# 1Jamie/HMSE

Hardware: AMD Instinct MI355X
Metric: ingest_GiB_per_s (higher is better)
Workload: dtype u8; 1 GPU; full ingest (FastCDC 2/8/32 KiB + SHA-256 dedupe + MinHash-128/LSH 4x32 + dictionary DEFLATE level-9 profile) over 10.00 GB wikipedia; total_bytes=9999220736, seg_size=4194304, collective=none

## Files before the change

hmse_amd/csrc/l1_deflate.hip:

```cpp
#include "common.h"
#include "blockops.h"
#include <stdio.h>
#include <stdlib.h>
#include <mutex>

namespace dfl {

constexpr int HB = 12;
constexpr int NBK = 1 << HB;
constexpr uint32_t MINM = 4, MAXM = 258, WMAX = 32768;

__device__ __forceinline__ uint32_t hash4(uint32_t x) { return (x * 0x9E3779B1u) >> (32 - HB); }

__device__ __forceinline__ uint32_t alignb(uint32_t hi, uint32_t lo, uint32_t sh) { return __builtin_amdgcn_alignbyte(hi, lo, sh); }
__device__ __forceinline__ uint32_t ld32a(const uint8_t* W, uint32_t off) {
  const uint32_t* w = (const uint32_t*)(W + (off & ~3u));
  return alignb(w[1], w[0], off);
}
__device__ __forceinline__ void ld64a(const uint8_t* W, uint32_t off, uint32_t& x0, uint32_t& x1) {
  const uint32_t* w = (const uint32_t*)(W + (off & ~3u));
  const uint32_t a = w[0], b = w[1], c = w[2];
  x0 = alignb(b, a, off); x1 = alignb(c, b, off);
}
__device__ __forceinline__ uint32_t sort_key(const uint8_t* W, uint32_t off) {
// ... 14 lines not shown
__device__ __forceinline__ uint32_t cur_get(const uint32_t* c, uint32_t h) { return (c[h >> 1] >> ((h & 1u) * 16u)) & 0xFFFFu; }
__device__ __forceinline__ uint32_t cur_inc(uint32_t* c, uint32_t h) {
  const uint32_t sh = (h & 1u) * 16u;
  return (atomicAdd(&c[h >> 1], 1u << sh) >> sh) & 0xFFFFu;
}

__device__ __forceinline__ void len_sym(uint32_t len, uint32_t& code, uint32_t& eb, uint32_t& ev) {
  if (len == 258) { code = 285; eb = 0; ev = 0; return; }
  const uint32_t l = len - 3;
  if (l < 8) { code = 257 + l; eb = 0; ev = 0; return; }
  const uint32_t e = (31 - __builtin_clz(l)) - 2;
  code = 257 + 4 * e + 4 + ((l >> e) & 3); eb = e; ev = l & ((1u << e) - 1);
}
__device__ __forceinline__ void dist_sym(uint32_t dist, uint32_t& code, uint32_t& eb, uint32_t& ev) {
  const uint32_t d = dist - 1;
  if (d < 4) { code = d; eb = 0; ev = 0; return; }
  const uint32_t hb = 31 - __builtin_clz(d), e = hb - 1;
  code = 2 * hb + ((d >> e) & 1); eb = e; ev = d & ((1u << e) - 1);
}
__device__ __forceinline__ uint32_t len_extra_bits(uint32_t code) {
  if (code < 265 || code == 285) return 0;
  return (code - 261) >> 2;
}
__device__ __forceinline__ uint32_t dist_extra_bits(uint32_t code) { return code < 4 ? 0 : (code >> 1) - 1; }
__device__ __forceinline__ uint32_t fixed_len(uint32_t s) { return s < 144 ? 8 : s < 256 ? 9 : s < 280 ? 7 : 8; }

__device__ __forceinline__ void wave_sync() {
  __builtin_amdgcn_fence(__ATOMIC_ACQ_REL, "wavefront");
  __builtin_amdgcn_wave_barrier();
}

template <int NT>
__device__ __forceinline__ uint32_t block_exclusive_scan_w(uint32_t v, uint32_t t, uint32_t* red, uint32_t* total) {
  const uint32_t lane = t & 63u, wave = uni32(t >> 6);
  const uint32_t inc = wave_incl_scan(v);
  if (lane == 63u) red[wave] = inc;
  __syncthreads();
  const uint32_t c = lane < (uint32_t)(NT / 64) ? red[lane] : 0u;
  const uint32_t ci = wave_incl_scan(c);
  __syncthreads();
  *total = (uint32_t)__builtin_amdgcn_readlane((int)ci, 63);
  return (uint32_t)__builtin_amdgcn_readlane((int)(ci - c), (int)wave) + inc - v;
}

template <int N>
struct HuffScratchT {
  uint32_t key[N];
  uint32_t sorted[N];
  uint32_t w[2 * N];
  uint16_t parent[2 * N];
  uint32_t cnt[32];
};
using HuffL = HuffScratchT<288>;
using HuffD = HuffScratchT<32>;

template <int NT, bool WQ>
struct Small {
  uint32_t lf[288], df[32];
  uint32_t red[NT / 64 + 1];
  uint32_t qhead;
  uint32_t ocnt[4];
  uint32_t otot[4];
  unsigned long long opk[1];
  struct { uint32_t ji, job, L, Dl; uint64_t c, cstart, rec_at, dstart; } nx;
  struct { uint64_t rec_at; } cur;
  uint32_t pexit[NT / 64], pexit2[NT / 64], pconv[NT / 64];
  uint8_t wtab[WQ ? NT : 64];
};

constexpr int align16(int v) { return (v + 15) & ~15; }

#ifndef HMSE_TCAP_S
#define HMSE_TCAP_S 10048
#define HMSE_TCAP_S2 13952
#define HMSE_TCAP_SG 17408
#define HMSE_TCAP_SG2 22976
#endif
constexpr int NT_S = 1024, TCAP_S = HMSE_TCAP_S, TCAP_S2 = HMSE_TCAP_S2, TCAP_SG = HMSE_TCAP_SG, TCAP_SG2 = HMSE_TCAP_SG2;
constexpr int NT_M = 1024, TCAP_SG3 = 32768;
#ifndef HMSE_NT_B
#define HMSE_NT_B 1024
#endif
constexpr int NT_B = HMSE_NT_B, TCAP_B = 65536, LCAP_B = 32768;

template <int NT, int TCAP, int LCAP_, bool LDSM, bool MDG = false, bool MLG = false, bool NOK = false>
struct Layout {
  static constexpr int LCAP = LCAP_;
  static constexpr int W_OFF = 0;
  static constexpr int W_SZ = align16(TCAP + 64);
  static constexpr int CUR_OFF = W_OFF + W_SZ;
  static constexpr int CUR_SZ = NBK * 2;
  static constexpr int MARK_OFF = CUR_OFF + CUR_SZ;
  static constexpr int MARK_SZ = align16(LCAP / 8 + 16);
  static constexpr int SMALL_OFF = MARK_OFF + MARK_SZ;
  static constexpr int SMALL_SZ = align16((int)sizeof(Small<NT, !LDSM>));
  static constexpr int A_OFF = SMALL_OFF + SMALL_SZ;
  static constexpr int A_SZ = LDSM ? align16(2 * TCAP + 80) : align16(LCAP + 80);
  static constexpr int MD_OFF = A_OFF + A_SZ;
  static constexpr int MD_SZ = (LDSM && !MDG) ? align16(2 * LCAP) : 0;
  static constexpr int ML_OFF = MD_OFF + MD_SZ;
  static constexpr int ML_SZ = (LDSM && !MLG) ? align16(LCAP) : 0;
  static constexpr int K_OFF = ML_OFF + ML_SZ;
  static constexpr int K_SZ = (LDSM && !NOK) ? align16(TCAP + 16) : 0;
  static constexpr int TOTAL = K_OFF + K_SZ;
  static_assert(TOTAL <= 160 * 1024, "one workgroup's LDS image must fit the CU's 160 KiB");
  static_assert(!(LDSM && TCAP <= TCAP_SG2) || TOTAL <= 80 * 1024, "classes S .. SG2 run two workgroups per CU");
  static_assert(sizeof(HuffL) + sizeof(HuffD) <= CUR_SZ, "Huffman scratch must fit the cursor table");
};

template <typename HS>
__device__ void huff_lengths_wave(const uint32_t* freq, uint32_t n, uint32_t limit, uint8_t* lens, HS* hs) {
  const uint32_t lane = lane_id();
  uint32_t used = 0;
  for (uint32_t b = 0; b < n; b += 64) {
    const uint32_t s = b + lane;
    used += (uint32_t)__builtin_popcountll(__ballot(s < n && freq[s] != 0));
  }
  uint32_t dummy0 = 0xFFFFFFFFu, dummy1 = 0xFFFFFFFFu;
  if (used == 0) { dummy0 = 0; dummy1 = 1; }
  else if (used == 1) dummy0 = freq[0] != 0 ? 1u : 0u;
  uint32_t m = 0;
  for (uint32_t b = 0; b < n; b += 64) {
    const uint32_t s = b + lane;
    uint32_t f = s < n ? freq[s] : 0u;
    if (s == dummy0 || s == dummy1) f = 1;
    if (s < n) lens[s] = 0;
    const bool u = f != 0;
    const uint64_t mask = __ballot(u);
    if (u) hs->key[m + (uint32_t)__builtin_popcountll(mask & lanemask_lt())] = (f << 9) | s;
    m += (uint32_t)__builtin_popcountll(mask);
  }
  wave_sync();
  for (uint32_t j = lane; j < m; j += 64) {
    const uint32_t kj = hs->key[j];
    uint32_t r = 0;
    for (uint32_t i = 0; i < m; i++) r += hs->key[i] < kj;
    hs->sorted[r] = kj;
    hs->w[r] = kj >> 9;
  }
  if (lane < 32) hs->cnt[lane] = 0;
  wave_sync();
  if (lane == 0) {
    constexpr uint32_t INF = 0xFFFFFFFFu;
    uint32_t li = 0, ii = m, ni = m;
    uint32_t wl = m ? hs->w[0] : INF, wi = INF;
    for (uint32_t step = 0; step + 1 < m; step++) {
      uint32_t pick0, pick1, v0, v1;
      {
        const bool tl = li < m && (ii >= ni || wl <= wi);
        if (tl) { pick0 = li++; v0 = wl; wl = li < m ? hs->w[li] : INF; }
        else { pick0 = ii++; v0 = wi; wi = ii < ni ? hs->w[ii] : INF; }
      }
      {
        const bool tl = li < m && (ii >= ni || wl <= wi);
        if (tl) { pick1 = li++; v1 = wl; wl = li < m ? hs->w[li] : INF; }
        else { pick1 = ii++; v1 = wi; wi = ii < ni ? hs->w[ii] : INF; }
      }
      hs->w[ni] = v0 + v1;
      hs->parent[pick0] = (uint16_t)ni; hs->parent[pick1] = (uint16_t)ni;
      if (ii == ni) wi = v0 + v1;
      ni++;
    }
  }
  wave_sync();
  const uint32_t root = 2 * m - 2;
  for (uint32_t j = lane; j < m; j += 64) {
// ... 34 lines not shown
#pragma unroll
  for (uint32_t b = 1; b <= 15; b++) { code = (code + (b > 1 ? uni32(cnt[b - 1]) : 0u)) << 1; run[b] = code; }
  for (uint32_t b0 = 0; b0 < n; b0 += 64) {
    const uint32_t s = b0 + lane;
    const uint32_t l = s < n ? lens[s] : 0u;
    uint32_t mycode = 0;
#pragma unroll
    for (uint32_t b = 1; b <= 15; b++) {
      const uint64_t mask = __ballot(l == b);
      if (l == b) mycode = run[b] + (uint32_t)__builtin_popcountll(mask & lanemask_lt());
      run[b] += (uint32_t)__builtin_popcountll(mask);
    }
    if (s < n) codes[s] = l ? (uint16_t)(__builtin_bitreverse32(mycode) >> (32 - l)) : (uint16_t)0;
  }
  wave_sync();
}

__device__ __forceinline__ void put_bits(uint32_t* out, uint32_t off, uint32_t v, uint32_t nb) {
  if (nb == 0) return;
  const uint32_t w = off >> 5, s = off & 31;
  atomicOr(&out[w], v << s);
  if (s + nb > 32) atomicOr(&out[w + 1], v >> (32 - s));
}

template <typename SM>
__device__ void rle_tree_wave(const uint8_t* l, uint32_t n, SM* sm, uint32_t tok_base, uint32_t* tok_end) {
  const uint32_t lane = lane_id();
  uint64_t starts[5];
  uint32_t val[5];
#pragma unroll
  for (int b = 0; b < 5; b++) {
    const uint32_t i = b * 64 + lane;
    const uint32_t v = i < n ? l[i] : 0xFFu;
    const uint32_t pv = (i > 0 && i < n) ? l[i - 1] : 0x1FFu;
    val[b] = v;
    starts[b] = __ballot(i < n && (i == 0 || v != pv));
  }
  uint32_t base = tok_base;
#pragma unroll
  for (int b = 0; b < 5; b++) {
    const uint32_t i = b * 64 + lane;
    const bool is_start = (starts[b] >> lane) & 1ull;
    uint32_t nxt = n;
    {
      bool found = false;
#pragma unroll
      for (int c = 0; c < 5; c++) {
        if (c < b) continue;
        uint64_t m = starts[c];
        if (c == b) m &= (lane == 63) ? 0ull : (~0ull << (lane + 1));
        if (!found && m) { nxt = c * 64 + (uint32_t)__builtin_ctzll(m); found = true; }
      }
    }
    const uint32_t v = val[b];
    uint32_t R = is_start ? nxt - i : 0u;
    uint32_t cnt = 0, full = 0, rem = 0;
    if (is_start) {
      if (v == 0) { full = R / 138; rem = R % 138; cnt = full + (rem >= 3 ? 1u : rem); }
      else { const uint32_t r1 = R - 1; full = r1 / 6; rem = r1 % 6; cnt = 1 + full + (rem >= 3 ? 1u : rem); }
    }
    const uint32_t inc = wave_incl_scan(cnt);
    const uint32_t tot = (uint32_t)__builtin_amdgcn_readlane((int)inc, 63);
    uint32_t at = base + inc - cnt;
    if (is_start) {
      if (v == 0) {
        for (uint32_t k = 0; k < full; k++) { sm->rle_sym[at] = 18; sm->rle_eb[at] = 7; sm->rle_ev[at] = 127; at++; }
        if (rem >= 11) { sm->rle_sym[at] = 18; sm->rle_eb[at] = 7; sm->rle_ev[at] = (uint8_t)(rem - 11); at++; }
        else if (rem >= 3) { sm->rle_sym[at] = 17; sm->rle_eb[at] = 3; sm->rle_ev[at] = (uint8_t)(rem - 3); at++; }
        else for (uint32_t k = 0; k < rem; k++) { sm->rle_sym[at] = 0; sm->rle_eb[at] = 0; sm->rle_ev[at] = 0; at++; }
      } else {
        sm->rle_sym[at] = (uint8_t)v; sm->rle_eb[at] = 0; sm->rle_ev[at] = 0; at++;
        for (uint32_t k = 0; k < full; k++) { sm->rle_sym[at] = 16; sm->rle_eb[at] = 2; sm->rle_ev[at] = 3; at++; }
        if (rem >= 3) { sm->rle_sym[at] = 16; sm->rle_eb[at] = 2; sm->rle_ev[at] = (uint8_t)(rem - 3); at++; }
        else for (uint32_t k = 0; k < rem; k++) { sm->rle_sym[at] = (uint8_t)v; sm->rle_eb[at] = 0; sm->rle_ev[at] = 0; at++; }
      }
    }
    base += tot;
  }
  *tok_end = base;
  wave_sync();
}

#ifdef HMSE_DFL_STAMPS
__device__ unsigned long long g_dfl_stamps[6][24];
__device__ unsigned long long g_enc_stamps[8];
#define STAMP(i) do { if (threadIdx.x == 0) { const unsigned long long now__ = clock64(); stamp_acc[i] += now__ - stamp_last; stamp_last = now__; } } while (0)
#else
#define STAMP(i) do { } while (0)
#endif

__host__ __device__ __forceinline__ uint32_t rec_ntok_off() { return 1280u; }
__host__ __device__ __forceinline__ uint32_t rec_tok_off() { return 1296u; }
__host__ __device__ __forceinline__ uint32_t rec_body(uint32_t L) { return 1296u + 4u * ((L + 3u) & ~3u); }
__host__ __device__ __forceinline__ uint32_t rec_slot_off(uint32_t L, uint32_t variant) { return variant ? rec_body(L) : rec_tok_off(); }
__host__ __device__ __forceinline__ uint32_t rec_size(uint32_t L, bool has_dict) { return (rec_body(L) + (has_dict ? L + 5u + 16u : 0u) + 255u) & ~255u; }

struct Args {
  const uint8_t* data; uint64_t n;
  const uint64_t* cuts; const uint64_t* chunk_ids; const int64_t* base; uint64_t n_sel;
  uint32_t depth;
  uint32_t base_is_chunk;
  const uint64_t* rec_off;
  uint8_t* recs;
  uint64_t rec_cap; uint32_t* status;
  uint32_t* len_full; uint32_t* len_delta;
  uint8_t* scratch; size_t scratch_stride;
  uint8_t* scratch2; size_t scratch2_stride;
  const uint32_t* jobs; const uint32_t* n_jobs; uint32_t* counter;
  unsigned long long* prof_ctr; uint32_t prof_slot;
};


typedef const __attribute__((address_space(4))) Args* KArgs;
__device__ __forceinline__ KArgs kargs() {
  KArgs p = (KArgs)__builtin_amdgcn_kernarg_segment_ptr();
  asm volatile("" : "+s"(p));
  return p;
}

struct Scratch {
  uint16_t S[65536]; uint8_t K[65536 + 16];
  uint16_t jumpA[32768 + 8];
};

template <int NT, int TCAP, int LCAP_, bool LDSM, bool MDG = false, bool MLG = false, bool NOK = false, bool DICT = false>
__global__ __launch_bounds__(NT, (LDSM ? (NT == 1024 && TCAP <= TCAP_SG2 ? 8 : 4) : 2)) void l1_deflate_kernel(Args) {
  using LY = Layout<NT, TCAP, LCAP_, LDSM, MDG, MLG, NOK>;
  constexpr int LCAP = LY::LCAP;
  extern __shared__ __attribute__((aligned(16))) uint8_t smem[];
  uint8_t* const W = smem + LY::W_OFF;
  uint32_t* const cur = (uint32_t*)(smem + LY::CUR_OFF);
  uint32_t* const mark = (uint32_t*)(smem + LY::MARK_OFF);
  Small<NT, !LDSM>& sm = *(Small<NT, !LDSM>*)(smem + LY::SMALL_OFF);
  auto scratch_wg = [&]() -> Scratch* { const KArgs a = kargs(); return (Scratch*)(a->scratch + (size_t)blockIdx.x * a->scratch_stride); };
  auto scratch2_wg = [&]() -> uint8_t* { const KArgs a = kargs(); return a->scratch2 + (size_t)blockIdx.x * a->scratch2_stride; };
  Scratch* const sc = LDSM ? nullptr : scratch_wg();
  uint16_t* const S = LDSM ? (uint16_t*)(smem + LY::A_OFF) : sc->S;
  uint16_t* const jump = LDSM ? (uint16_t*)(smem + LY::A_OFF) : sc->jumpA;
  uint8_t* const K = LDSM ? (uint8_t*)(smem + LY::K_OFF) : sc->K;
  auto n_jobs_now = [&]() -> uint32_t { return *kargs()->n_jobs; };
#if defined(HMSE_NO_ORD) || defined(HMSE_NO_SORT_ORD)
  constexpr bool SORT_ORD = false;
#else
  constexpr bool SORT_ORD = LDSM && !MLG && !DICT;
#endif
#if defined(HMSE_NO_ORD) || defined(HMSE_NO_DICT_ORD) || defined(HMSE_NO_DICT_POSLIST)
  constexpr bool POS_ORD = false;
#else
  constexpr bool POS_ORD = LDSM && DICT;
#endif
  static_assert(!POS_ORD || TCAP < 65536, "a rank waits in a match-distance slot");
  static_assert(!SORT_ORD || LY::ML_SZ >= NBK * 2, "the bucket starts wait in the match-length area during the sort");
  [[maybe_unused]] uint32_t* const starts = (uint32_t*)(smem + LY::ML_OFF);
#ifdef HMSE_DFL_STAMPS
  unsigned long long stamp_acc[24] = {0}, stamp_last = clock64();
#endif

  auto pf_fetch_sync = [&]() {
    const KArgs a = kargs();
    const uint32_t ji2 = atomicAdd(a->counter, 1u);
    sm.nx.ji = ji2;
    if (ji2 >= *a->n_jobs) return;
    const uint32_t job2 = a->jobs[ji2];
    const uint64_t k2 = job2 >> 1;
    const uint64_t c2 = a->chunk_ids ? a->chunk_ids[k2] : k2;
    const uint64_t cs = a->cuts[c2];
    sm.nx.job = job2; sm.nx.c = c2; sm.nx.cstart = cs; sm.nx.L = (uint32_t)(a->cuts[c2 + 1] - cs); sm.nx.rec_at = a->rec_off[k2];
    if constexpr (DICT) {
      const int64_t bsel = a->base[k2];
      const uint64_t bc = (a->chunk_ids && !a->base_is_chunk) ? a->chunk_ids[bsel] : (uint64_t)bsel;
      uint64_t ds = a->cuts[bc], dl = a->cuts[bc + 1] - ds;
      if (dl > WMAX) { ds += dl - WMAX; dl = WMAX; }
      sm.nx.dstart = ds; sm.nx.Dl = (uint32_t)dl;
    }
  };
  if (threadIdx.x == 0) pf_fetch_sync();
  for (;;) {
    uint32_t t = threadIdx.x;
    asm volatile("" : "+v"(t));
    const uint32_t lane = t & 63u, wave = t >> 6;
    __syncthreads();
    const uint32_t ji = uni32(sm.nx.ji);
    if (ji >= n_jobs_now()) break;
    STAMP(10);
    constexpr uint32_t variant = DICT ? 1u : 0u;
    const uint32_t L = uni32(sm.nx.L);
    const uint32_t Dl = variant ? uni32(sm.nx.Dl) : 0u;
    const uint32_t T = Dl + L;
    uint32_t pf_u = 0; uint64_t pf_a = 0, pf_b = 0, pf_c = 0;
    auto pf_stage = [&](int stg) {
      const KArgs a = kargs();
      const uint32_t n_jobs = *a->n_jobs;
      const bool valid = stg <= 1 || sm.nx.ji < n_jobs;
      switch (stg) {
        case 0: pf_u = atomicAdd(a->counter, 1u); break;
        case 1: sm.nx.ji = pf_u; pf_u = pf_u < n_jobs ? a->jobs[pf_u] : 0u; break;
        case 2: {
          sm.nx.job = pf_u;
          if (valid) { const uint64_t k2 = pf_u >> 1; pf_a = a->chunk_ids ? a->chunk_ids[k2] : k2; pf_b = a->rec_off[k2]; if (DICT) pf_c = (uint64_t)a->base[k2]; }
          break;
        }
        case 3: sm.nx.c = pf_a; sm.nx.rec_at = pf_b; if (DICT) sm.nx.dstart = pf_c; break;
        case 4:
          if (valid) {
            const uint64_t c2 = sm.nx.c;
            pf_a = a->cuts[c2]; pf_b = a->cuts[c2 + 1];
            if (DICT) { const uint64_t bsel = sm.nx.dstart; pf_c = (a->chunk_ids && !a->base_is_chunk) ? a->chunk_ids[bsel] : bsel; }
          }
          break;
        case 5:
          sm.nx.cstart = pf_a; sm.nx.L = (uint32_t)(pf_b - pf_a);
          if (DICT && valid) { const uint64_t bc = pf_c; pf_a = a->cuts[bc]; pf_b = a->cuts[bc + 1]; }
          break;
        default:
          if (DICT && valid) { uint64_t ds = pf_a, dl = pf_b - pf_a; if (dl > WMAX) { ds += dl - WMAX; dl = WMAX; } sm.nx.dstart = ds; sm.nx.Dl = (uint32_t)dl; }
          break;
      }
    };
#define PF_STAGE(n) do { if (t == 0) pf_stage(n); } while (0)
    auto mdist_of = [&]() -> uint16_t* { if constexpr (LDSM && !MDG) return (uint16_t*)(smem + LY::MD_OFF); else return (uint16_t*)scratch2_wg(); };
    auto mlen_of = [&]() -> uint8_t* { if constexpr (LDSM && !MLG) return (uint8_t*)(smem + LY::ML_OFF); else return scratch2_wg() + 2u * (uint32_t)LCAP; };
    {
      const KArgs a = kargs();
      const uint64_t rec_at = uni64(sm.nx.rec_at);
      if (L > (uint32_t)LCAP || T > (uint32_t)TCAP || rec_at + (uint64_t)rec_size(L, variant != 0) > a->rec_cap) {
        if (t == 0) {
          const uint64_t k = sm.nx.job >> 1;
          (variant ? a->len_delta : a->len_full)[k] = 0xFFFFFFFFu;
          if (L <= 32768u) atomicOr(a->status, 2u);
        }
        __syncthreads();
        if (t == 0) pf_fetch_sync();
        continue;
      }
      if (t == 0) sm.cur.rec_at = rec_at;
    }
    const uint8_t* const csrc = kargs()->data + uni64(sm.nx.cstart);
    const uint8_t* const dsrc = kargs()->data + (variant ? uni64(sm.nx.dstart) : 0ull);
// ... 73 lines not shown
    STAMP(1);
    PF_STAGE(1);
    {
      static_assert(!SORT_ORD || TCAP < 65536, "16-bit list cursors");
      [[maybe_unused]] const uint16_t* const start_of = (const uint16_t*)starts;
      uint32_t q = t, h = 0, before = 0, hx = 0;
      [[maybe_unused]] uint32_t bidx = 0;
      bool act = q < nh;
      if (act) {
        hx = sort_key(W, q); h = hx >> (32 - HB); before = cur_get(cur, h);
        if constexpr (SORT_ORD) bidx = before - start_of[h];
      }
      [[maybe_unused]] uint32_t* ord = nullptr;
      [[maybe_unused]] uint32_t dcap = 0, ob1 = 0, ob2 = 0, ob3 = 0;
      if constexpr (SORT_ORD) {
        ord = (uint32_t*)(scratch2_wg() + 98304u);
        dcap = __builtin_elementwise_min(kargs()->depth, 63u);
        ob1 = uni32(sm.otot[0]); ob2 = ob1 + uni32(sm.otot[1]); ob3 = ob2 + uni32(sm.otot[2]);
      }
      [[maybe_unused]] uint16_t* rank_at = nullptr;
      if constexpr (POS_ORD) rank_at = mdist_of();
      __syncthreads();
      for (uint32_t q0 = 0; q0 < nh; q0 += NT) {
        if (act) S[cur_inc(cur, h)] = (uint16_t)q;
        __syncthreads();
        uint32_t r = 0;
        if (act) {
          const uint32_t after = cur_get(cur, h);
          for (uint32_t jj = before; jj < after; jj++) r += S[jj] < q;
        }
        [[maybe_unused]] uint32_t km = 0, obl = 0, obh = 0;
        [[maybe_unused]] uint64_t oc0 = 0, oc1 = 0, oc2 = 0, oc3 = 0;
        if constexpr (SORT_ORD) {
          km = bidx + r;
          km = km < dcap ? km : dcap;
          oc0 = __ballot(km >= 24u); oc1 = __ballot(km >= 12u); oc2 = __ballot(km >= 4u); oc3 = __ballot(km >= 1u);
          if (oc3 != 0 && lane == 0u) {
            uint32_t z = 0;
            asm volatile("" : "+v"(z));
            const unsigned long long got = atomicAdd(&sm.opk[z], (unsigned long long)__builtin_popcountll(oc0) | ((unsigned long long)__builtin_popcountll(oc1 & ~oc0) << 16) |
                                                                     ((unsigned long long)__builtin_popcountll(oc2 & ~oc1) << 32) | ((unsigned long long)__builtin_popcountll(oc3 & ~oc2) << 48));
            obl = (uint32_t)got; obh = (uint32_t)(got >> 32);
          }
        }
        const uint32_t qn = q0 + NT + t;
        const bool actn = qn < nh;
        uint32_t hn = 0, beforen = 0, hxn = 0;
        [[maybe_unused]] uint32_t bidxn = 0;
        if (actn) {
          hxn = sort_key(W, qn); hn = hxn >> (32 - HB); beforen = cur_get(cur, hn);
          if constexpr (SORT_ORD) bidxn = beforen - start_of[hn];
        }
        __syncthreads();
        if (act) { S[before + r] = (uint16_t)q; if constexpr (!NOK) K[before + r] = (uint8_t)((hx & 0x0Fu) | ((hx >> 12) & 0xF0u)); }
        if constexpr (POS_ORD) if (act && q >= Dl) *(uint16_t*)((uint8_t*)rank_at + ((q - Dl) << 1)) = (uint16_t)(before + r);
        if constexpr (SORT_ORD) {
          if (oc3 != 0) {
            const uint32_t gl = (uint32_t)__builtin_amdgcn_readlane((int)obl, 0), gh = (uint32_t)__builtin_amdgcn_readlane((int)obh, 0);
            uint32_t pos = 0;
            if (km >= 1u) { pos = ob3 + (gh >> 16) + mbcnt64(oc3 & ~oc2); asm volatile("" : "+v"(pos)); }
            if (km >= 4u) { pos = ob2 + (gh & 0xFFFFu) + mbcnt64(oc2 & ~oc1); asm volatile("" : "+v"(pos)); }
            if (km >= 12u) { pos = ob1 + (gl >> 16) + mbcnt64(oc1 & ~oc0); asm volatile("" : "+v"(pos)); }
            if (km >= 24u) { pos = (gl & 0xFFFFu) + mbcnt64(oc0); asm volatile("" : "+v"(pos)); }
            if (km != 0u) *(uint32_t*)((uint8_t*)ord + (pos << 2)) = (before + r) | (km << 15) | ((hx << 5) & 0x01E00000u);
          }
          bidx = bidxn;
        }
        q = qn; act = actn; h = hn; before = beforen; hx = hxn;
      }
      if constexpr (SORT_ORD) for (uint32_t i = t * 16; i < L; i += NT * 16) *(uint4*)(mlen0 + i) = make_uint4(0, 0, 0, 0);
      __syncthreads();
#ifdef HMSE_DIAG
      if constexpr (SORT_ORD) if (t < 4u && (uint32_t)((sm.opk[0] >> (16u * t)) & 0xFFFFull) != sm.otot[t]) atomicOr(kargs()->status, 32u);
#endif
    }
    STAMP(2);
    PF_STAGE(2);
    uint32_t* const anch = mark;
    uint8_t* const anchb = (uint8_t*)(mark + (LCAP / 64 + 2));
    static_assert(LCAP % 64 == 0 && (LCAP / 64 + 2) * 4 + LCAP / 64 + 2 <= LY::MARK_SZ, "anchors and their backward extents share the mark area");
    if constexpr (DICT) {
      const uint32_t n_anch = (L + 63u) >> 6;
      if (t < 2u) { anch[n_anch + t] = 0; anchb[n_anch + t] = 0; }
      for (uint32_t a0 = wave; a0 < n_anch; a0 += NT / 64) {
        const uint32_t pa = Dl + (a0 << 6);
        uint32_t word = 0, back = 0;
        if (pa + 4 <= T) {
          const uint32_t h = hash4(ld32a(W, pa));
          const uint32_t lo = h ? cur_get(cur, h - 1) : 0u, hi = cur_get(cur, h);
          uint32_t l = lo, r = hi;
          while (l < r) { const uint32_t m = (l + r) >> 1; if ((uint32_t)S[m] < Dl) l = m + 1; else r = m; }
          const uint32_t first = l > lo + 64u ? l - 64u : lo;
          const uint32_t idx = first + lane;
          uint32_t ml = 0, q = 0;
          if (idx < l) {
            q = S[idx];
            if (TCAP <= (int)WMAX || pa - q <= WMAX) {
              uint64_t qa[4], pb[4];
              ldNa<4>(W, q, qa); ldNa<4>(W, pa, pb);
              ml = 32;
#pragma unroll
              for (int u = 3; u >= 0; u--) { const uint64_t x = qa[u] ^ pb[u]; if (x) ml = 8u * u + ((uint32_t)__builtin_ctzll(x) >> 3); }
            }
          }
          uint32_t key = (ml << 8) | lane;
          key = wave_max(key);
          if ((key >> 8) >= 32u) {
            const uint32_t d = pa - (uint32_t)__builtin_amdgcn_readlane((int)q, (int)(key & 63u));
            const uint32_t off = 8u * lane;
            uint32_t n = 8;
            if (pa + off < T) {
              uint64_t xa[1], xb[1];
              ldNa<1>(W, pa + off - d, xa); ldNa<1>(W, pa + off, xb);
              const uint64_t x = xa[0] ^ xb[0];
              if (x) n = (uint32_t)__builtin_ctzll(x) >> 3;
            } else n = 0;
            const uint64_t mm = __ballot(n < 8u);
            uint32_t run = 512;
            if (mm) { const uint32_t fl = (uint32_t)__builtin_ctzll(mm); run = 8u * fl + (uint32_t)__builtin_amdgcn_readlane((int)n, (int)fl); }
            if (run > T - pa) run = T - pa;
            word = d | (run << 16);
            const uint32_t qa0 = pa - d;
            uint32_t nb = 8;
            if (lane < 16u) {
              nb = 0;
              if (qa0 >= off + 8u) {
                uint64_t ya[1], yb[1];
                ldNa<1>(W, qa0 - off - 8u, ya); ldNa<1>(W, pa - off - 8u, yb);
                const uint64_t y = ya[0] ^ yb[0];
                nb = y ? (uint32_t)__builtin_clzll(y) >> 3 : 8u;
              }
            }
            const uint64_t mb = __ballot(nb < 8u);
            back = 128;
            if (mb) {
              const uint32_t fl = (uint32_t)__builtin_ctzll(mb);
              const uint64_t n0 = __ballot((nb & 1u) != 0), n1 = __ballot((nb & 2u) != 0), n2 = __ballot((nb & 4u) != 0);
              back = 8u * fl + (uint32_t)((n0 >> fl) & 1ull) + 2u * (uint32_t)((n1 >> fl) & 1ull) + 4u * (uint32_t)((n2 >> fl) & 1ull);
            }
            if (back > (a0 << 6)) back = a0 << 6;
          }
        }
        anch[a0] = word; anchb[a0] = (uint8_t)back;
      }
      __syncthreads();
      STAMP(22);
    }
    auto hint_of = [&](uint32_t p, uint32_t maxlen, uint32_t& bq) -> uint32_t {
      const uint32_t a0 = (p - Dl) >> 6;
      uint32_t bm = 0; bq = 0;
#pragma unroll
      for (uint32_t back = 0; back < 2; back++) {
        if (a0 < back) continue;
        const uint32_t w = anch[a0 - back];
        const uint32_t d = w & 0xFFFFu, run = w >> 16, pa = Dl + ((a0 - back) << 6);
        if (w == 0 || p < pa || d > p || p - d >= Dl) continue;
        uint32_t m = 0;
        if (run >= 512u) m = maxlen;
        else if (pa + run > p) m = (pa + run - p) < maxlen ? (pa + run - p) : maxlen;
        if (m > bm) { bm = m; bq = p - d; }
      }
      return bm;
    };
    [[maybe_unused]] auto hint_word = [&](uint32_t p, uint32_t maxlen, uint32_t w, uint32_t pa, uint32_t& bm, uint32_t& bq) {
      const uint32_t d = w & 0xFFFFu, run = w >> 16;
      if (w == 0 || p < pa || d > p || p - d >= Dl) return;
      uint32_t m = 0;
      if (run >= 512u) m = maxlen;
      else if (pa + run > p) m = (pa + run - p) < maxlen ? (pa + run - p) : maxlen;
      if (m > bm) { bm = m; bq = p - d; }
    };
    [[maybe_unused]] auto known_of = [&](uint32_t p, uint32_t maxlen) -> uint32_t {
      const uint32_t a1 = ((p - Dl) >> 6) + 1u;
      uint32_t kf = 0;
#pragma unroll
      for (uint32_t f = 0; f < 2; f++) {
        const uint32_t w = anch[a1 + f], bk = anchb[a1 + f], pa = Dl + ((a1 + f) << 6);
        if (pa - p <= bk) {
          const uint32_t d = w & 0xFFFFu, run = w >> 16;
          uint32_t m = pa + run - p;
          if (run >= 512u || m > maxlen) m = maxlen;
          const uint32_t v = (p - d) | (m << 16);
          if (v > kf) kf = v;
        }
      }
      return kf;
    };
    if constexpr (DICT && !POS_ORD) {
      uint8_t* const mlen = mlen_of(); uint16_t* const mdist = mdist_of();
      for (uint32_t x = t; x < L; x += NT) {
        const uint32_t p = Dl + x;
        if (p + 4 > T) continue;
        const uint32_t maxlen = (T - p) < MAXM ? (T - p) : MAXM;
        uint32_t bq;
        const uint32_t bm = hint_of(p, maxlen, bq);
        if (bm >= 16u) { mlen[x] = (uint8_t)(bm - 3); mdist[x] = (uint16_t)(p - bq); }
      }
      if constexpr (!MLG && LDSM) __syncthreads();
      STAMP(23);
    }
#if defined(HMSE_NO_ORD)
    constexpr bool ORD = false;
#elif defined(HMSE_NO_DICT_ORD)
    constexpr bool ORD = !DICT && LDSM;
#else
    constexpr bool ORD = LDSM;
#endif
    auto ord_of = [&]() -> uint32_t* { return (uint32_t*)(scratch2_wg() + 98304u); };
    if constexpr (ORD && !SORT_ORD) {
      const uint32_t depth = kargs()->depth;
      uint32_t* const ord = ord_of();
      constexpr int ITER = (TCAP + NT - 1) / NT;
      const uint32_t wv = uni32(wave);
      constexpr int NPK = (ITER + 2) / 3;
      uint32_t pk[NPK];
#pragma unroll
      for (int w = 0; w < NPK; w++) pk[w] = 0;
      uint32_t n0 = 0, n1 = 0, n2 = 0, n3 = 0;
      if constexpr (!POS_ORD) {
        const uint32_t last = nh ? nh - 1u : 0u;
        constexpr int G = DICT ? 2 : ITER > 12 ? 4 : 8;
        [[maybe_unused]] const uint8_t* const mlen_h = mlen_of();
#pragma unroll
        for (int g = 0; g < ITER; g += G) if ((uint32_t)g * NT < nh) {
          uint32_t pv[G], hv[G], lv[G];
#pragma unroll
          for (int u = 0; u < G; u++) if (g + u < ITER) { const uint32_t r = (wv << 6) + (uint32_t)(g + u) * NT + lane; pv[u] = S[r < last ? r : last]; }
#pragma unroll
          for (int u = 0; u < G; u++) if (g + u < ITER) hv[u] = ld32a(W, pv[u]) * 0x9E3779B1u;
// ... 499 lines not shown
          mark[wb >> 5] = (uint32_t)m; mark[(wb >> 5) + 1] = (uint32_t)(m >> 32);
        }
        conv_out = conv;
        return conv ? chain_exit : curp;
      };
      {
        const uint32_t sw = wave * SEG;
        bool conv = true;
        uint32_t ex = sm.pexit[wave];
        if (wave > 0 && sw < L) ex = stitch(wave, sm.pexit[wave - 1], sm.pexit[wave], true, conv);
        wave_sync();
        sm.pexit2[wave] = ex; sm.pconv[wave] = (wave == 0 || sw >= L || conv) ? 1u : 0u;
      }
      __syncthreads();
      if (wave == 0) {
        uint32_t first_bad = NW;
        for (uint32_t w = 0; w < NW; w++) if (sm.pconv[w] == 0u) { first_bad = w; break; }
        if (first_bad < NW) {
          uint32_t tru = sm.pexit2[first_bad];
          for (uint32_t w = first_bad + 1; w < NW; w++) {
            if (w * SEG >= L) break;
            bool cv;
            tru = stitch(w, tru, sm.pexit2[w], false, cv);
          }
        }
      }
    }
    __syncthreads();
    STAMP(4);
    PF_STAGE(6);
    {
      const KArgs a = kargs();
      uint8_t* const rec_c = a->recs + uni64(sm.cur.rec_at);
      const uint16_t* const mdist_c = mdist_of();
      uint32_t* const tok = (uint32_t*)(rec_c + rec_tok_off());
      const uint32_t ppt = (L + NT - 1) / NT;
      const uint32_t p0 = t * ppt < L ? t * ppt : L, p1 = (p0 + ppt) < L ? (p0 + ppt) : L;
      auto bits_at = [&](uint32_t pos, uint32_t nb) -> uint32_t {
        const uint32_t w = pos >> 5;
        const uint64_t v = (uint64_t)mark[w] | ((uint64_t)mark[w + 1] << 32);
        return (uint32_t)(v >> (pos & 31u)) & (nb >= 32u ? 0xFFFFFFFFu : ((1u << nb) - 1u));
      };
      uint32_t cntm = 0;
      for (uint32_t pos = p0; pos < p1; pos += 32) cntm += (uint32_t)__builtin_popcount(bits_at(pos, p1 - pos));
      uint32_t ntok;
      uint32_t idx = block_exclusive_scan_w<NT>(cntm, t, sm.red, &ntok);
      for (uint32_t pos = p0; pos < p1; pos += 32) {
        uint32_t m = bits_at(pos, p1 - pos);
        while (m) {
          const uint32_t x = pos + (uint32_t)__builtin_ctz(m);
          m &= m - 1;
          uint32_t l3 = 0;
          bool tk;
          if constexpr (LDSM) { const uint32_t nxj = jump[x]; tk = nxj > x + 1u; l3 = nxj - x - 3u; }
          else { tk = take(x); if (tk) l3 = mlen_c[x]; }
          if (tk) {
            const uint32_t dd = mdist_c[x];
            uint32_t code, eb, ev;
            len_sym(l3 + 3u, code, eb, ev); atomicAdd(&sm.lf[code], 1u);
            dist_sym(dd, code, eb, ev); atomicAdd(&sm.df[code], 1u);
            tok[idx] = (256u + l3) | (dd << 16);
          } else {
            const uint32_t b = W[Dl + x];
            atomicAdd(&sm.lf[b], 1u);
            tok[idx] = b;
          }
          idx++;
        }
      }
      if (t == 0) { atomicAdd(&sm.lf[256], 1u); *(uint32_t*)(rec_c + rec_ntok_off()) = ntok; if (a->prof_ctr) atomicAdd(&a->prof_ctr[a->prof_slot], (unsigned long long)ntok); }
      __syncthreads();
      STAMP(5);
      uint32_t* const r_hist = (uint32_t*)rec_c;
      for (uint32_t i = t; i < 288; i += NT) r_hist[i] = sm.lf[i];
      if (t < 32) r_hist[288 + t] = sm.df[t];
    }
    STAMP(9);
#ifdef HMSE_DFL_STAMPS
    if (t == 0) { stamp_acc[14] += L; stamp_acc[15]++; }
#endif
  }
#undef PF_STAGE
#ifdef HMSE_DFL_STAMPS
  if (threadIdx.x == 0) for (int i = 0; i < 24; i++) atomicAdd(&g_dfl_stamps[(TCAP <= TCAP_S ? 0 : TCAP <= TCAP_SG ? 1 : 2) + (DICT ? 3 : 0)][i], stamp_acc[i]);
#endif
}


struct EncSmall {
  uint32_t lf[288], df[32], cf[20];
  uint8_t ll[288], dl[32], cl[20];
  uint16_t lc[288], dc[32], cc[20];
  uint8_t rle_sym[352], rle_eb[352], rle_ev[352];
  uint32_t nr, nlit, ndist, ncl, mode, hdr_bits, fixed_bits, extra_bits, data_bits, cl_bits;
  uint32_t job, spill;
};
template <int LMIN_, int LCAP_>
struct EncLayout {
  static constexpr int NT = 128, LMIN = LMIN_, LCAP = LCAP_;
  static constexpr int NB_MAX = (LCAP + 63) / 64;
  static constexpr int NBLK = (NB_MAX + 1 + 63) / 64;
  static constexpr int SMALL_OFF = 0;
  static constexpr int SMALL_SZ = align16((int)sizeof(EncSmall));
  static constexpr int HS_OFF = SMALL_OFF + SMALL_SZ;
  static constexpr int HS_SZ = align16((int)(sizeof(HuffL) + sizeof(HuffD)));
  static constexpr int TT_OFF = HS_OFF;
  static constexpr int OUT_OFF = TT_OFF + 2048;
  static constexpr int WIN_BYTES = 4096;
  static constexpr int OUT_SZ = HS_SZ - 2048;
  static constexpr bool BOFF_IN_LF = NB_MAX + 1 <= 288;
  static constexpr int BOFF_OFF = HS_OFF + HS_SZ;
  static constexpr int BOFF_SZ = BOFF_IN_LF ? 0 : align16(4 * (NB_MAX + 1));
  static constexpr int TOTAL = BOFF_OFF + BOFF_SZ;
  static_assert(OUT_SZ >= WIN_BYTES + 64, "window + overhang");
  static_assert(LCAP > 12288 || TOTAL <= 10240, "sixteen workgroups per CU for the records of chunks <= 12 KiB");
};

template <int LMIN, int LCAP>
__global__ __launch_bounds__(128, 8) void l1_encode_kernel(Args a, const bool force_spill) {
  using EL = EncLayout<LMIN, LCAP>;
  constexpr uint32_t NT = EL::NT;
  constexpr uint32_t WIN_BITS = EL::WIN_BYTES * 8;
  extern __shared__ __attribute__((aligned(16))) uint8_t smem[];
  EncSmall& sm = *(EncSmall*)(smem + EL::SMALL_OFF);
  HuffL* const hsL = (HuffL*)(smem + EL::HS_OFF);
  HuffD* const hsD = (HuffD*)(smem + EL::HS_OFF + sizeof(HuffL));
  uint32_t* const TT = (uint32_t*)(smem + EL::TT_OFF);
  uint32_t* const out = (uint32_t*)(smem + EL::OUT_OFF);
  uint32_t* const boff = EL::BOFF_IN_LF ? sm.lf : (uint32_t*)(smem + EL::BOFF_OFF);
  const uint32_t n_jobs = *a.n_jobs;
#ifdef HMSE_DFL_STAMPS
  unsigned long long e_acc0 = 0, e_acc1 = 0, e_acc2 = 0, e_acc3 = 0, e_acc4 = 0, e_acc5 = 0, e_n = 0, e_last = clock64();
#define ESTAMP(v) do { if (threadIdx.x == 0) { const unsigned long long now__ = clock64(); v += now__ - e_last; e_last = now__; } } while (0)
#else
#define ESTAMP(v) do { } while (0)
#endif
  for (;;) {
  uint32_t t = threadIdx.x;
  asm volatile("" : "+v"(t));
  const uint32_t lane = t & 63u, wave = uni32(t >> 6);
  __syncthreads();
  if (t == 0) sm.job = atomicAdd(a.counter, 1u);
  __syncthreads();
  const uint32_t ji = uni32(sm.job);
  if (ji >= n_jobs) break;
  const uint32_t job = uni32(a.jobs[ji]);
  const uint64_t k = job >> 1;
  const uint32_t variant = job & 1u;
  const uint64_t c = a.chunk_ids ? uni64(a.chunk_ids[k]) : k;
  const uint64_t cstart = uni64(a.cuts[c]);
  const uint32_t L = uni32((uint32_t)(a.cuts[c + 1] - cstart));
  if (L <= (uint32_t)LMIN || L > (uint32_t)LCAP) continue;
  uint32_t* len_out = variant ? a.len_delta : a.len_full;
  if (uni32(len_out[k]) == 0xFFFFFFFFu) continue;
  uint8_t* const rec = a.recs + uni64(a.rec_off[k]);
  const uint32_t* const r_hist = (const uint32_t*)rec;
  const uint32_t ntok = uni32(*(const uint32_t*)(rec + rec_ntok_off()));
  const uint32_t* const tok = (const uint32_t*)(rec + rec_tok_off());
  if (a.prof_ctr && t == 0) atomicAdd(&a.prof_ctr[a.prof_slot], (unsigned long long)ntok);
  uint8_t* const slot = rec + rec_slot_off(L, variant);
  const uint8_t* const lit = a.data + cstart;
  for (uint32_t i = t; i < 288; i += NT) sm.lf[i] = r_hist[i];
  if (t < 32) sm.df[t] = r_hist[288 + t];
  if (t < 20) sm.cf[t] = 0;
  __syncthreads();
  ESTAMP(e_acc0);
  if (wave == 0) huff_lengths_wave(sm.lf, 286, 15, sm.ll, hsL);
// ... 372 lines not shown
  if (n_dev) n = *n_dev;
  __shared__ unsigned long long s[SC_NT / 64];
  const uint64_t i = (uint64_t)blockIdx.x * SC_NT + threadIdx.x;
  unsigned long long v = i < n ? in[i] : 0ull;
  for (int d = 32; d > 0; d >>= 1) v += __shfl_down(v, d, 64);
  if (lane_id() == 0) s[threadIdx.x >> 6] = v;
  __syncthreads();
  if (threadIdx.x == 0) { unsigned long long tt = 0; for (int w = 0; w < SC_NT / 64; w++) tt += s[w]; bsum[blockIdx.x] = tt; }
}
__global__ __launch_bounds__(SC_NT) void scan_apply_kernel(const uint64_t* __restrict__ in, uint64_t n, const uint64_t* __restrict__ bsum,
                                                            uint64_t* __restrict__ out, const uint64_t* __restrict__ n_dev) {
  if (n_dev) n = *n_dev;
  __shared__ unsigned long long s[SC_NT / 64];
  const uint64_t i = (uint64_t)blockIdx.x * SC_NT + threadIdx.x;
  const unsigned long long v = i < n ? in[i] : 0ull;
  const unsigned long long inc = wave_incl_scan((uint64_t)v);
  if (lane_id() == 63) s[threadIdx.x >> 6] = inc;
  __syncthreads();
  unsigned long long wb = 0;
  for (uint32_t w = 0; w < (threadIdx.x >> 6); w++) wb += s[w];
  if (i < n) out[i] = bsum[blockIdx.x] + wb + inc - v;
  if (i + 1 == n) out[n] = bsum[blockIdx.x] + wb + inc;
}

static int exclusive_scan_u64(const uint64_t* in, uint64_t n, uint64_t* out, uint64_t* bsum, uint64_t* total, hipStream_t stream,
                              const uint64_t* n_dev = nullptr) {
  const uint64_t nb = (n + SC_NT - 1) / SC_NT;
  scan_reduce_kernel<<<dim3((uint32_t)nb), dim3(SC_NT), 0, stream>>>(in, n, bsum, n_dev);
  block_sums_scan_kernel<SC_NT, 0, uint64_t, SC_NT><<<dim3(1), dim3(SC_NT), 0, stream>>>(bsum, nb, total, n_dev);
  scan_apply_kernel<<<dim3((uint32_t)nb), dim3(SC_NT), 0, stream>>>(in, n, bsum, out, n_dev);
  return hipGetLastError() == hipSuccess ? HMSE_OK : HMSE_EHIP;
}

constexpr int N_WG_B = 256;

struct Ws {
  uint32_t* counters;
  uint64_t* rec_off; uint64_t* final_len; uint64_t* bsum; uint64_t* rec_total;
  uint32_t* len_full; uint32_t* len_delta; uint32_t* lists; uint64_t list_stride;
  uint8_t* scratch; uint8_t* scratch2; uint8_t* recs; size_t fixed_bytes;
};
static Ws carve(void* ws, uint64_t n_sel) {
  WsCarver w(ws, ~(size_t)0);
  Ws r;
  r.counters = w.take<uint32_t>(N_CTR);
  r.rec_total = w.take<uint64_t>(1);
  r.rec_off = w.take<uint64_t>(n_sel + 1);
  r.final_len = w.take<uint64_t>(n_sel + 1);
  r.bsum = w.take<uint64_t>((n_sel + SC_NT - 1) / SC_NT + 1);
  r.len_full = w.take<uint32_t>(n_sel);
  r.len_delta = w.take<uint32_t>(n_sel);
  r.list_stride = 2 * n_sel;
  r.lists = w.take<uint32_t>(N_LIST * r.list_stride);
  r.scratch = w.take<uint8_t>((size_t)N_WG_B * hmse_align_up(sizeof(Scratch), 256));
  r.scratch2 = w.take<uint8_t>((size_t)512 * hmse_align_up(8 * 32768, 256));
  r.fixed_bytes = w.off;
  r.recs = r.scratch ? (uint8_t*)ws + w.off : nullptr;
  return r;
}

template <bool DICT, int NT, int TCAP, int LCAP, bool LDSM, bool MDG = false, bool MLG = false, bool NOK = false>
static int launch_class(Args a, uint32_t grid, hipStream_t stream) {
  using LY = Layout<NT, TCAP, LCAP, LDSM, MDG, MLG, NOK>;
  static std::once_flag attr_once;
  static hipError_t attr_rc = hipSuccess;
  std::call_once(attr_once, [] {
    attr_rc = hipFuncSetAttribute((const void*)l1_deflate_kernel<NT, TCAP, LCAP, LDSM, MDG, MLG, NOK, DICT>, hipFuncAttributeMaxDynamicSharedMemorySize, LY::TOTAL);
  });
  if (attr_rc != hipSuccess) return HMSE_EHIP;
  l1_deflate_kernel<NT, TCAP, LCAP, LDSM, MDG, MLG, NOK, DICT><<<dim3(grid), dim3(NT), LY::TOTAL, stream>>>(a);
  return hipGetLastError() == hipSuccess ? HMSE_OK : HMSE_EHIP;
}

}

#ifdef HMSE_DFL_STAMPS
extern "C" int hmse_debug_encode_stamps(unsigned long long* out8, int reset) {
  if (hipMemcpyFromSymbol(out8, HIP_SYMBOL(dfl::g_enc_stamps), sizeof(dfl::g_enc_stamps)) != hipSuccess) return HMSE_EHIP;
  if (reset) { unsigned long long z[8] = {0}; if (hipMemcpyToSymbol(HIP_SYMBOL(dfl::g_enc_stamps), z, sizeof z) != hipSuccess) return HMSE_EHIP; }
  return HMSE_OK;
}
extern "C" int hmse_debug_deflate_stamps(unsigned long long* out96, int reset) {
  if (hipMemcpyFromSymbol(out96, HIP_SYMBOL(dfl::g_dfl_stamps), sizeof(dfl::g_dfl_stamps)) != hipSuccess) return HMSE_EHIP;
  if (reset) { unsigned long long z[144] = {0}; if (hipMemcpyToSymbol(HIP_SYMBOL(dfl::g_dfl_stamps), z, sizeof z) != hipSuccess) return HMSE_EHIP; }
  return HMSE_OK;
}
#endif

extern "C" uint64_t hmse_l1_deflate_record_bytes(uint32_t chunk_len) { return chunk_len <= 32768u ? dfl::rec_size(chunk_len, false) : 0u; }
extern "C" uint64_t hmse_l1_deflate_record_bytes_dict(uint32_t chunk_len) { return chunk_len <= 32768u ? dfl::rec_size(chunk_len, true) : 0u; }

size_t hmse_l1_deflate_workspace_bytes_impl(uint64_t n_sel, const hmse_cfg*) { return dfl::carve(nullptr, n_sel).fixed_bytes; }

static int deflate_impl(const uint8_t* data, uint64_t n, const uint64_t* cuts, const uint64_t* chunk_ids,
                        const int64_t* base, uint64_t n_sel, const uint64_t* n_dev, const uint64_t* out_base_dev, const hmse_cfg* cfg, uint32_t flags,
                        uint8_t* out, uint64_t out_cap, uint64_t* out_off, uint8_t* kind, uint32_t* status, void* ws, size_t ws_bytes,
                        void* stream_);

extern "C" int hmse_l1_deflate_ex(const uint8_t* data, uint64_t n, const uint64_t* cuts, const uint64_t* chunk_ids,
                                  const int64_t* base, uint64_t n_sel, const hmse_cfg* cfg, uint32_t flags, uint8_t* out,
                                  uint64_t out_cap, uint64_t* out_off, uint8_t* kind, uint32_t* status, void* ws, size_t ws_bytes,
                                  void* stream_) {
  return deflate_impl(data, n, cuts, chunk_ids, base, n_sel, nullptr, nullptr, cfg, flags, out, out_cap, out_off, kind, status, ws, ws_bytes, stream_);
}

int hmse_l1_deflate_dyn(const uint8_t* data, uint64_t n_cap, const uint64_t* cuts_all, const uint64_t* sel_ids, const int64_t* sel_base,
                        const uint64_t* n_sel_dev, uint64_t cap_sel, const uint64_t* out_base_dev, const hmse_cfg* cfg, uint8_t* out, uint64_t out_cap,
                        uint64_t* out_off, uint8_t* kind, uint32_t* status, void* ws, size_t ws_bytes, hipStream_t stream) {
  if (!n_sel_dev || cap_sel == 0) return HMSE_EINVAL;
  return deflate_impl(data, n_cap, cuts_all, sel_ids, sel_base, cap_sel, n_sel_dev, out_base_dev, cfg, HMSE_DEFLATE_BASE_IS_CHUNK_ID, out, out_cap, out_off,
                      kind, status, ws, ws_bytes, (void*)stream);
}

static int deflate_impl(const uint8_t* data, uint64_t n, const uint64_t* cuts, const uint64_t* chunk_ids,
                        const int64_t* base, uint64_t n_sel, const uint64_t* n_dev, const uint64_t* out_base_dev, const hmse_cfg* cfg, uint32_t flags,
                        uint8_t* out, uint64_t out_cap, uint64_t* out_off, uint8_t* kind, uint32_t* status, void* ws, size_t ws_bytes,
                        void* stream_) {
  HMSE_WS_ALIGNED(ws);
  using namespace dfl;
  if (hmse_cfg_validate_impl(cfg) != 0) return HMSE_EINVAL;
  if (flags & ~(uint32_t)HMSE_DEFLATE_BASE_IS_CHUNK_ID) return HMSE_EINVAL;
  const uint32_t a_base_is_chunk = (flags & HMSE_DEFLATE_BASE_IS_CHUNK_ID) ? 1u : 0u;
  if (!out_off || !status) return HMSE_EINVAL;
  hipStream_t stream = (hipStream_t)stream_;
  (void)hipGetLastError();
  HMSE_FILL(status, 0, sizeof(uint32_t), stream);
  if (n_sel == 0) { HMSE_FILL(out_off, 0, sizeof(uint64_t), stream); return HMSE_OK; }
  if (!data || !cuts || !out || !kind) return HMSE_EINVAL;
  if (n_sel > 0x3FFFFFFFull) return HMSE_EINVAL;
  Ws w = carve(ws, n_sel);
  if (!ws || ws_bytes < w.fixed_bytes) return HMSE_ENOSPC;
  const uint64_t avail = ws_bytes - w.fixed_bytes;
  HMSE_FILL(w.counters, 0, N_CTR * sizeof(uint32_t), stream);
  HMSE_FILL(w.len_full, 0, n_sel * sizeof(uint32_t), stream);
  HMSE_FILL(w.len_delta, 0, n_sel * sizeof(uint32_t), stream);
  const uint32_t blocks = (uint32_t)((n_sel + 255) / 256);
  rec_size_kernel<<<dim3(blocks), dim3(256), 0, stream>>>(cuts, chunk_ids, base, n_sel, w.rec_off, n_dev);
  HMSE_LAUNCH_CHECK();
  if (exclusive_scan_u64(w.rec_off, n_sel, w.rec_off, w.bsum, w.rec_total, stream, n_dev) != HMSE_OK) return HMSE_EHIP;
  classify_kernel<<<dim3((uint32_t)((n_sel + LIST_NT - 1) / LIST_NT)), dim3(LIST_NT), 0, stream>>>(cuts, chunk_ids, base, n_sel, a_base_is_chunk, w.lists, w.list_stride, w.counters, n_dev);
  HMSE_LAUNCH_CHECK();
  Args a;
  a.data = data; a.n = n; a.cuts = cuts; a.chunk_ids = chunk_ids; a.base = base; a.n_sel = n_sel;
  a.depth = hmse_deflate_depth(cfg);
  a.base_is_chunk = a_base_is_chunk;
  a.rec_off = w.rec_off; a.recs = w.recs; a.len_full = w.len_full; a.len_delta = w.len_delta;
  a.rec_cap = avail; a.status = status;
  a.scratch = w.scratch; a.scratch_stride = hmse_align_up(sizeof(Scratch), 256);
  a.scratch2 = w.scratch2; a.scratch2_stride = hmse_align_up(8 * 32768, 256);
  const uint64_t max_jobs = 2 * n_sel;
  auto sel = [&](int c) { a.jobs = w.lists + (size_t)c * w.list_stride; a.n_jobs = w.counters + c; a.counter = w.counters + 32 + c; };
  static const bool dbg_sync = getenv("HMSE_DFL_DEBUG_SYNC") != nullptr;
  auto dbg = [&](int slot) { if (dbg_sync) { const hipError_t e = hipStreamSynchronize(stream); fprintf(stderr, "[hmse_l1_deflate] launch of slot %d finished (%d)\n", slot, (int)e); fflush(stderr); } };
  a.prof_ctr = g_hmse_prof ? g_hmse_prof_ctr : nullptr; a.prof_slot = 0;
  static const bool enc_force_spill = getenv("HMSE_ENC_FORCE_SPILL") != nullptr;
#define HMSE_DFL_LAUNCH(DICT_, LIST, SLOT, GRID, ...)                                                               \
  sel(LIST); a.prof_slot = (SLOT);                                                                                   \
  PROF_BEGIN(SLOT, stream);                                                                                          \
  if (launch_class<DICT_, __VA_ARGS__>(a, (uint32_t)(max_jobs < (uint64_t)(GRID) ? max_jobs : (uint64_t)(GRID)), stream) != HMSE_OK) return HMSE_EHIP; \
  PROF_END(SLOT, stream); dbg(SLOT);
#define HMSE_DFL_ENCODE(LIST1, SLOT1, LIST2, SLOT2)                                                                  \
  sel(LIST1); a.prof_slot = (SLOT1);                                                                                 \
  PROF_BEGIN(SLOT1, stream);                                                                                         \
  l1_encode_kernel<0, 12288><<<dim3((uint32_t)(max_jobs < 4096 ? max_jobs : 4096)), dim3(128), EncLayout<0, 12288>::TOTAL, stream>>>(a, enc_force_spill);           \
  PROF_END(SLOT1, stream); dbg(SLOT1);                                                                               \
  sel(LIST2); a.prof_slot = (SLOT2);                                                                                 \
  PROF_BEGIN(SLOT2, stream);                                                                                         \
// ... 40 lines not shown
```

Measured before the change: 34.73 GiB/s.

## Split dictionary anchor search into staged bucket scan, grouped verify, and run pass

Dictionary anchor discovery used to run one anchor per wavefront, doing a binary search, a 64-lane candidate compare and the run extension all in one pass. It now runs in three stages. First, one thread per anchor finds the bucket range. Second, sub-wave groups of ANCH_GW lanes verify candidates newest-first and stop at the first 32-byte match. Third, each wave computes forward and backward runs only for anchors that found a match. The aim is to spread the search work across more lanes and skip idle wavefronts on anchors with no match. The cost is two extra block barriers and possibly different candidate selection, which is checked under the diagnostics build.

Result: faster. 35.32 GiB/s (median of 6 runs) (+1.7%).

```diff
diff --git a/hmse_amd/csrc/l1_deflate.hip b/hmse_amd/csrc/l1_deflate.hip
--- a/hmse_amd/csrc/l1_deflate.hip
+++ b/hmse_amd/csrc/l1_deflate.hip
@@ -120,6 +120,11 @@
 #define HMSE_NT_B 1024
 #endif
 constexpr int NT_B = HMSE_NT_B, TCAP_B = 65536, LCAP_B = 32768;
+#ifndef HMSE_ANCH_GW
+#define HMSE_ANCH_GW 16
+#endif
+constexpr uint32_t ANCH_GW = HMSE_ANCH_GW;
+static_assert(ANCH_GW >= 8u && ANCH_GW <= 64u && (ANCH_GW & (ANCH_GW - 1u)) == 0u, "a wavefront holds a whole number of groups");
 
 template <int NT, int TCAP, int LCAP_, bool LDSM, bool MDG = false, bool MLG = false, bool NOK = false>
 struct Layout {
@@ -320,7 +325,8 @@
 }
 
 #ifdef HMSE_DFL_STAMPS
-__device__ unsigned long long g_dfl_stamps[6][24];
+constexpr int N_STAMPS = 26;
+__device__ unsigned long long g_dfl_stamps[6][N_STAMPS];
 __device__ unsigned long long g_enc_stamps[8];
 #define STAMP(i) do { if (threadIdx.x == 0) { const unsigned long long now__ = clock64(); stamp_acc[i] += now__ - stamp_last; stamp_last = now__; } } while (0)
 #else
@@ -391,7 +397,7 @@
   static_assert(!SORT_ORD || LY::ML_SZ >= NBK * 2, "the bucket starts wait in the match-length area during the sort");
   [[maybe_unused]] uint32_t* const starts = (uint32_t*)(smem + LY::ML_OFF);
 #ifdef HMSE_DFL_STAMPS
-  unsigned long long stamp_acc[24] = {0}, stamp_last = clock64();
+  unsigned long long stamp_acc[N_STAMPS] = {0}, stamp_last = clock64();
 #endif
 
   auto pf_fetch_sync = [&]() {
@@ -631,6 +637,7 @@
     if constexpr (DICT) {
       const uint32_t n_anch = (L + 63u) >> 6;
       if (t < 2u) { anch[n_anch + t] = 0; anchb[n_anch + t] = 0; }
+#if defined(HMSE_NO_ANCH_STAGES)
       for (uint32_t a0 = wave; a0 < n_anch; a0 += NT / 64) {
         const uint32_t pa = Dl + (a0 << 6);
         uint32_t word = 0, back = 0;
@@ -694,6 +701,146 @@
       }
       __syncthreads();
       STAMP(22);
+#else
+      auto anchor_runs = [&](uint32_t pa, uint32_t a0, uint32_t d, uint32_t& word, uint32_t& back) {
+        const uint32_t off = 8u * lane;
+        uint32_t n = 8;
+        if (pa + off < T) {
+          uint64_t xa[1], xb[1];
+          ldNa<1>(W, pa + off - d, xa); ldNa<1>(W, pa + off, xb);
+          const uint64_t x = xa[0] ^ xb[0];
+          if (x) n = (uint32_t)__builtin_ctzll(x) >> 3;
+        } else n = 0;
+        const uint64_t mm = __ballot(n < 8u);
+        uint32_t run = 512;
+        if (mm) { const uint32_t fl = (uint32_t)__builtin_ctzll(mm); run = 8u * fl + (uint32_t)__builtin_amdgcn_readlane((int)n, (int)fl); }
+        if (run > T - pa) run = T - pa;
+        word = d | (run << 16);
+        const uint32_t qa0 = pa - d;
+        uint32_t nb = 8;
+        if (lane < 16u) {
+          nb = 0;
+          if (qa0 >= off + 8u) {
+            uint64_t ya[1], yb[1];
+            ldNa<1>(W, qa0 - off - 8u, ya); ldNa<1>(W, pa - off - 8u, yb);
+            const uint64_t y = ya[0] ^ yb[0];
+            nb = y ? (uint32_t)__builtin_clzll(y) >> 3 : 8u;
+          }
+        }
+        const uint64_t mb = __ballot(nb < 8u);
+        back = 128;
+        if (mb) {
+          const uint32_t fl = (uint32_t)__builtin_ctzll(mb);
+          const uint64_t n0 = __ballot((nb & 1u) != 0), n1 = __ballot((nb & 2u) != 0), n2 = __ballot((nb & 4u) != 0);
+          back = 8u * fl + (uint32_t)((n0 >> fl) & 1ull) + 2u * (uint32_t)((n1 >> fl) & 1ull) + 4u * (uint32_t)((n2 >> fl) & 1ull);
+        }
+        if (back > (a0 << 6)) back = a0 << 6;
+      };
+      [[maybe_unused]] auto anchor_wave = [&](uint32_t a0, uint32_t& word, uint32_t& back) {
+        const uint32_t pa = Dl + (a0 << 6);
+        word = 0; back = 0;
+        if (pa + 4 <= T) {
+          const uint32_t h = hash4(ld32a(W, pa));
+          const uint32_t lo = h ? cur_get(cur, h - 1) : 0u, hi = cur_get(cur, h);
+          uint32_t l = lo, r = hi;
+          while (l < r) { const uint32_t m = (l + r) >> 1; if ((uint32_t)S[m] < Dl) l = m + 1; else r = m; }
+          const uint32_t first = l > lo + 64u ? l - 64u : lo;
+          const uint32_t idx = first + lane;
+          uint32_t ml = 0, q = 0;
+          if (idx < l) {
+            q = S[idx];
+            if (TCAP <= (int)WMAX || pa - q <= WMAX) {
+              uint64_t qa[4], pb[4];
+              ldNa<4>(W, q, qa); ldNa<4>(W, pa, pb);
+              ml = 32;
+#pragma unroll
+              for (int u = 3; u >= 0; u--) { const uint64_t x = qa[u] ^ pb[u]; if (x) ml = 8u * u + ((uint32_t)__builtin_ctzll(x) >> 3); }
+            }
+          }
+          uint32_t key = (ml << 8) | lane;
+          key = wave_max(key);
+          if ((key >> 8) >= 32u) {
+            const uint32_t d = pa - (uint32_t)__builtin_amdgcn_readlane((int)q, (int)(key & 63u));
+            anchor_runs(pa, a0, d, word, back);
+          }
+        }
+      };
+      {
+        const uint32_t wv = uni32(wave);
+        static_assert(LCAP / 64 < NT, "one lane per anchor in one trip");
+        if (const uint32_t a = t; a < n_anch) {
+          const uint32_t pa = Dl + (a << 6);
+          uint32_t v = 0;
+          if (pa + 4 <= T) {
+            const uint32_t h = hash4(ld32a(W, pa));
+            const uint32_t lo = h ? cur_get(cur, h - 1) : 0u, hi = cur_get(cur, h);
+            uint32_t l = lo, r = hi;
+            while (l < r) { const uint32_t m = (l + r) >> 1; if ((uint32_t)S[m] < Dl) l = m + 1; else r = m; }
+            const uint32_t cnt = l - lo < 64u ? l - lo : 64u;
+            v = cnt ? l | (cnt << 16) : 0u;
+          }
+          anch[a] = v;
+        }
+        __syncthreads();
+        STAMP(22);
+        {
+          constexpr uint32_t GW = ANCH_GW, GPW = 64u / GW;
+          const uint32_t g = lane / GW, j = lane % GW;
+          for (uint32_t ab = wv * GPW; ab < n_anch; ab += (uint32_t)(NT / 64) * GPW) {
+            const bool mine = ab + g < n_anch;
+            const uint32_t a = mine ? ab + g : ab;
+            const uint32_t v = mine ? anch[a] : 0u;
+            const uint32_t l = v & 0xFFFFu, cnt = v >> 16;
+            if (mine && j == 0u) anch[a] = 0;
+            if (__ballot(cnt != 0u) == 0ull) continue;
+            const uint32_t pa = Dl + (a << 6);
+            uint64_t pb[4];
+            ldNa<4>(W, pa, pb);
+            bool open = true;
+            for (uint32_t k = j; __ballot(open && k < cnt) != 0ull; k += GW) {
+              bool eq = false;
+              uint32_t q = 0;
+              if (open && k < cnt) {
+                q = S[l - 1u - k];
+                if (TCAP <= (int)WMAX || pa - q <= WMAX) {
+                  uint64_t qa[4];
+                  ldNa<4>(W, q, qa);
+                  eq = (((qa[0] ^ pb[0]) | (qa[1] ^ pb[1])) | ((qa[2] ^ pb[2]) | (qa[3] ^ pb[3]))) == 0ull;
+                }
+              }
+              const uint64_t m = __ballot(eq);
+              if constexpr (GW < 64u) {
+                const uint32_t gb = (uint32_t)(m >> (lane & ~(GW - 1u))) & (uint32_t)((1ull << GW) - 1ull);
+                if (gb != 0u) {
+                  if (eq && j == (uint32_t)__builtin_ctz(gb)) anch[a] = pa - q;
+                  open = false;
+                }
+              } else if (m != 0ull) {
+                if (eq && j == (uint32_t)__builtin_ctzll(m)) anch[a] = pa - q;
+                open = false;
+              }
+            }
+          }
+        }
+        __syncthreads();
+        STAMP(24);
+        for (uint32_t a0 = wv; a0 < n_anch; a0 += NT / 64) {
+          const uint32_t d = uni32(anch[a0]);
+          uint32_t word = 0, back = 0;
+          if (d != 0u) anchor_runs(Dl + (a0 << 6), a0, d, word, back);
+          anch[a0] = word; anchb[a0] = (uint8_t)back;
+        }
+        __syncthreads();
+        STAMP(25);
+#ifdef HMSE_DIAG
+        for (uint32_t a0 = wv; a0 < n_anch; a0 += NT / 64) {
+          uint32_t word, back;
+          anchor_wave(a0, word, back);
+          if (lane == 0u && (anch[a0] != word || anchb[a0] != (uint8_t)back)) atomicOr(kargs()->status, 64u);
+        }
+#endif
+      }
+#endif
     }
     auto hint_of = [&](uint32_t p, uint32_t maxlen, uint32_t& bq) -> uint32_t {
       const uint32_t a0 = (p - Dl) >> 6;
@@ -1359,7 +1506,7 @@
   }
 #undef PF_STAGE
 #ifdef HMSE_DFL_STAMPS
-  if (threadIdx.x == 0) for (int i = 0; i < 24; i++) atomicAdd(&g_dfl_stamps[(TCAP <= TCAP_S ? 0 : TCAP <= TCAP_SG ? 1 : 2) + (DICT ? 3 : 0)][i], stamp_acc[i]);
+  if (threadIdx.x == 0) for (int i = 0; i < N_STAMPS; i++) atomicAdd(&g_dfl_stamps[(TCAP <= TCAP_S ? 0 : TCAP <= TCAP_SG ? 1 : 2) + (DICT ? 3 : 0)][i], stamp_acc[i]);
 #endif
 }
 
@@ -1898,7 +2045,7 @@
 }
 extern "C" int hmse_debug_deflate_stamps(unsigned long long* out96, int reset) {
   if (hipMemcpyFromSymbol(out96, HIP_SYMBOL(dfl::g_dfl_stamps), sizeof(dfl::g_dfl_stamps)) != hipSuccess) return HMSE_EHIP;
-  if (reset) { unsigned long long z[144] = {0}; if (hipMemcpyToSymbol(HIP_SYMBOL(dfl::g_dfl_stamps), z, sizeof z) != hipSuccess) return HMSE_EHIP; }
+  if (reset) { unsigned long long z[6 * dfl::N_STAMPS] = {0}; if (hipMemcpyToSymbol(HIP_SYMBOL(dfl::g_dfl_stamps), z, sizeof z) != hipSuccess) return HMSE_EHIP; }
   return HMSE_OK;
 }
 #endif
```
